# ilya16/MultINN

Hardware: AMD Instinct MI355X
Metric: piano-roll timesteps/sec (train step), 5-track LSTM-NADE (higher is better)
Workload: dtype fp16; 1 GPU; TGT joint LSTM-NADE [1024,256,88,5]; global_batch=1024, per_gpu_batch=1024, seq_len=256, pitches=88, tracks=5, nade_hidden=256, optimizer=TF-Adam lr 0.01 eps 1e-4 clip 5.0, parallelism=dp1

## Files before the change

multinn_amd/csrc/nade_mfma.hip:

```cpp
#include "common.h"
#include "lstm_handoff.h"
typedef float nm_f4 __attribute__((ext_vector_type(4)));
#define NM_ST4(dst, a) __builtin_nontemporal_store((nm_f4){a[0], a[1], a[2], a[3]}, reinterpret_cast<nm_f4*>(dst))
#define NM_ST1(dst, x) __builtin_nontemporal_store((float)(x), dst)
#include <algorithm>
#include <type_traits>

typedef __bf16 bf16x8_t __attribute__((ext_vector_type(8)));
typedef float f32x4_t __attribute__((ext_vector_type(4)));
typedef __attribute__((address_space(1))) const void* gas_ptr_t;
typedef __attribute__((address_space(3))) void* lds_ptr_t;

#ifdef NM_TRACE
__device__ long long nm_trace[16];
#define NM_T(k) do { if (tid == 0 && blockIdx.x == NM_TRACE) { const long long now_ = wall_clock64(); nm_trace[k] += now_ - tprev_; tprev_ = now_; } } while (0)
#else
#define NM_T(k) do { } while (0)
#endif
#define NADE_EPS 1e-6f
#define LN2F 0.6931471805599453f
#define NM_H 256
#define NM_PITCH 264
#define NM_LP 36

__device__ __forceinline__ float nm_ln(float x) { return __builtin_amdgcn_logf(x) * LN2F; }

typedef _Float16 f16x8_t __attribute__((ext_vector_type(8)));
struct NmPairB { f16x8_t hi, lo; };
template <bool SPLIT> struct NmState;
template <> struct NmState<false> { typedef bf16_t T; static constexpr int PITCH = NM_PITCH; };
template <> struct NmState<true> { typedef unsigned T; static constexpr int PITCH = 260; };
__device__ __forceinline__ unsigned nm_pack_hl(float x) {
    const float hi = __uint_as_float(__float_as_uint(x) & 0xFFFFE000u);
    return __builtin_bit_cast(unsigned, __builtin_amdgcn_cvt_pkrtz(hi, x - hi));
}

template <bool SPLIT>
struct NadeFwdSmemT {
    float sA[SPLIT ? 1 : 32][NM_H];
    typename NmState<SPLIT>::T sH[32][NmState<SPLIT>::PITCH];
    typename NmState<SPLIT>::T sF[32][NmState<SPLIT>::PITCH];
    float sLb[32][NM_LP];
    float sLf[32][NM_LP];
    unsigned sMask[2][32];
    unsigned sSb[2][33];
    unsigned short sFl[2][1024];
    unsigned short sPs[2][34];
    unsigned sAct[2][32];
};

__device__ __forceinline__ void nm_load_a(const bf16_t (*tile)[NM_PITCH], int mi, int lane, bf16x8_t (&a)[8]) {
    const bf16_t* p = &tile[16 * mi + (lane & 15)][8 * (lane >> 4)];
#pragma unroll
    for (int s = 0; s < 8; ++s) a[s] = *reinterpret_cast<const bf16x8_t*>(p + 32 * s);
}
template <bool SPLIT> __device__ __forceinline__ typename NmState<SPLIT>::T nm_state(float h) {
    if constexpr (SPLIT) return nm_pack_hl(h);
    else return f32_to_bf16(h);
}
__device__ __forceinline__ f32x4_t nm_dot(const bf16x8_t (&af)[8], const bf16x8_t (&bfr)[8]) {
    f32x4_t acc = {0.f, 0.f, 0.f, 0.f};
#pragma unroll
    for (int s = 0; s < 8; ++s) acc = __builtin_amdgcn_mfma_f32_16x16x32_bf16(af[s], bfr[s], acc, 0, 0, 0);
    return acc;
}
__device__ __forceinline__ f32x4_t nm_dot_hl(const unsigned (*tile)[260], int mi, int lane, const NmPairB (&bw)[8]) {
    const unsigned* p = &tile[16 * mi + (lane & 15)][8 * (lane >> 4)];
    f32x4_t accm = {0.f, 0.f, 0.f, 0.f}, accs = {0.f, 0.f, 0.f, 0.f};
#pragma unroll
    for (int s = 0; s < 8; ++s) {
        const uint4 q0 = *reinterpret_cast<const uint4*>(p + 32 * s), q1 = *reinterpret_cast<const uint4*>(p + 32 * s + 4);
        uint4 uh, ul;
        uh.x = __builtin_amdgcn_perm(q0.y, q0.x, 0x05040100u); ul.x = __builtin_amdgcn_perm(q0.y, q0.x, 0x07060302u);
        uh.y = __builtin_amdgcn_perm(q0.w, q0.z, 0x05040100u); ul.y = __builtin_amdgcn_perm(q0.w, q0.z, 0x07060302u);
        uh.z = __builtin_amdgcn_perm(q1.y, q1.x, 0x05040100u); ul.z = __builtin_amdgcn_perm(q1.y, q1.x, 0x07060302u);
        uh.w = __builtin_amdgcn_perm(q1.w, q1.z, 0x05040100u); ul.w = __builtin_amdgcn_perm(q1.w, q1.z, 0x07060302u);
        const f16x8_t ah = __builtin_bit_cast(f16x8_t, uh), al = __builtin_bit_cast(f16x8_t, ul);
        accs = __builtin_amdgcn_mfma_f32_16x16x32_f16(ah, bw[s].lo, accs, 0, 0, 0);
        accm = __builtin_amdgcn_mfma_f32_16x16x32_f16(ah, bw[s].hi, accm, 0, 0, 0);
        accs = __builtin_amdgcn_mfma_f32_16x16x32_f16(al, bw[s].hi, accs, 0, 0, 0);
    }
    return accm + accs;
}
template <bool SPLIT, typename Tile, typename B>
__device__ __forceinline__ void nm_logit_tile(const Tile& tile, int w, int lane, const B& bfr, float (*out)[NM_LP]) {
    const int ni = w >> 1, mi = w & 1;
    f32x4_t acc;
    if constexpr (SPLIT) {
        acc = nm_dot_hl(tile, mi, lane, bfr);
    } else {
        bf16x8_t af[8];
        nm_load_a(tile, mi, lane, af);
        acc = nm_dot(af, bfr);
    }
#pragma unroll
    for (int i = 0; i < 4; ++i) out[16 * mi + 4 * (lane >> 4) + i][16 * ni + (lane & 15)] = acc[i];
}

template <bool SPLIT>
__device__ __forceinline__ void
nade_fwd_mfma_body(int tracks, int N, int D, const uint8_t* __restrict__ v, long v_track_stride, const float* __restrict__ bias, int ld_bias,
                     const float* __restrict__ w_enc, const bf16_t* __restrict__ w_dec_bf, const float* __restrict__ row_weight,
                     float* __restrict__ nll, float* __restrict__ cond_p, float* __restrict__ d_bias, float* __restrict__ a_final,
                     const int* __restrict__ gate, int run_if, const int* __restrict__ n_rows_dev) {
    extern __shared__ __attribute__((aligned(16))) char smem_raw[];
    typedef NadeFwdSmemT<SPLIT> NadeFwdSmem;
    typedef typename NmState<SPLIT>::T state_t;
    typedef typename std::conditional<SPLIT, NmPairB, bf16x8_t>::type bfrag_t;
    constexpr int KS = 8;
    NadeFwdSmem& S = *reinterpret_cast<NadeFwdSmem*>(smem_raw);
    if (gate != nullptr && *gate != run_if) return;
    constexpr int Hn = NM_H;
    const int m = blockIdx.y;
    const int tid = threadIdx.x, lane = tid & 63, w = __builtin_amdgcn_readfirstlane(tid >> 6);
    const int ni = w >> 1;
    const int rb = blockIdx.x * 32;
    const uint8_t* __restrict__ vm = v + (size_t)m * v_track_stride;
    const float* __restrict__ we = w_enc + (size_t)m * D * Hn;
    const bf16_t* __restrict__ wd = w_dec_bf + (size_t)m * D * Hn * (SPLIT ? 2 : 1);
    const int bd_off = tracks * Hn + m * D;
    const int ntile = (D + 31) / 32;
    if (n_rows_dev != nullptr && rb >= *n_rows_dev) {
        if (d_bias != nullptr)
            for (int e = tid; e < 32 * D; e += 256) {
                const int n = e / D, i = e - n * D;
                if (rb + n < N) d_bias[(size_t)(rb + n) * ld_bias + bd_off + i] = 0.f;
            }
        if (nll != nullptr && tid < 32 && rb + tid < N) nll[(size_t)m * N + rb + tid] = 0.f;
        return;
    }

    float areg[SPLIT ? 32 : 1];
    {
        float av[32];
#pragma unroll
        for (int n = 0; n < 32; ++n) av[n] = bias[(size_t)min(rb + n, N - 1) * ld_bias + m * Hn + tid];
#pragma unroll
        for (int n = 0; n < 32; ++n) {
            const float x = rb + n < N ? av[n] : 0.f;
            if constexpr (SPLIT) areg[n] = x;
            else S.sA[n][tid] = x;
            S.sH[n][tid] = nm_state<SPLIT>(fast_sigmoid(x));
        }
    }
    auto load_v = [&](int c, unsigned char (&vb)[4]) {
#pragma unroll
        for (int i = 0; i < 4; ++i) {
            const int row = min(rb + 8 * w + 2 * i + (lane >> 5), N - 1), dd = min(32 * c + (lane & 31), D - 1);
            vb[i] = vm[(size_t)row * D + dd];
        }
    };
    auto ballots = [&](int c, const unsigned char (&vb)[4], unsigned (&msk)[32]) {
#pragma unroll
        for (int i = 0; i < 4; ++i) {
            const int row = rb + 8 * w + 2 * i + (lane >> 5), dd = 32 * c + (lane & 31);
            const unsigned long long bal = __ballot(row < N && dd < D && vb[i] != 0);
            if (lane == 0) { msk[8 * w + 2 * i] = (unsigned)bal; msk[8 * w + 2 * i + 1] = (unsigned)(bal >> 32); }
        }
    };
    auto build_list = [&](int buf) {
        if (w == 0) {
            const unsigned mk = lane < 32 ? S.sMask[buf][lane] : 0u;
            const int cnt = __popc(mk);
            unsigned rest = mk;
            int base = 0;
            for (int j = 0; j < 32; ++j) {
                const unsigned act = (unsigned)__ballot(cnt > j);
                if (lane == 0) { S.sPs[buf][j] = (unsigned short)base; S.sAct[buf][j] = act; }
                if (act == 0u) break;
                if (cnt > j) {
                    const int pos = base + __popc(act & ((1u << lane) - 1u));
                    const int dpos = __builtin_ctz(rest);
                    rest &= rest - 1;
                    S.sFl[buf][pos] = (unsigned short)((lane << 5) | dpos);
                }
                base += __popc(act);
            }
            if (lane == 0) S.sSb[buf][32] = (unsigned)base;
        }
    };
    auto load_b = [&](int c, bfrag_t (&b)[KS]) {
        const int d = min(32 * c + 16 * ni + (lane & 15), D - 1);
        if constexpr (SPLIT) {
            const f16_t* p = reinterpret_cast<const f16_t*>(wd) + (size_t)d * 2 * Hn + 8 * (lane >> 4);
#pragma unroll
            for (int s = 0; s < KS; ++s) {
                b[s].hi = *reinterpret_cast<const f16x8_t*>(p + 32 * s);
                b[s].lo = *reinterpret_cast<const f16x8_t*>(p + Hn + 32 * s);
            }
        } else {
            const bf16_t* p = wd + (size_t)d * Hn + 8 * (lane >> 4);
#pragma unroll
            for (int s = 0; s < KS; ++s) b[s] = *reinterpret_cast<const bf16x8_t*>(p + 32 * s);
        }
    };
    const __amdgpu_buffer_rsrc_t we_rs = __builtin_amdgcn_make_buffer_rsrc(const_cast<float*>(we), 0, D * Hn * 4, 0x00020000);
    auto load_we = [&](int c, int buf, int k0, float (&wv)[32]) {
        const int F = (int)S.sSb[buf][32];
        const int entv = (int)S.sFl[buf][(k0 + (lane & 31) < F) ? k0 + (lane & 31) : 0];
#pragma unroll
        for (int u = 0; u < 32; ++u) {
            const int e = __builtin_amdgcn_readlane(entv, u);
            wv[u] = __builtin_bit_cast(float, __builtin_amdgcn_raw_buffer_load_b32(we_rs, tid * 4, min(32 * c + (e & 31), D - 1) * (Hn * 4), 0));
        }
    };
    unsigned char vb[4];
    bfrag_t bfr[KS];
    float wev[32];
    load_v(0, vb);
    load_b(0, bfr);
    ballots(0, vb, S.sMask[0]);
    if (ntile > 1) load_v(1, vb);
    __syncthreads();
    build_list(0);
    __syncthreads();
    load_we(0, 0, 0, wev);

    const int en = tid >> 3, ed0 = 4 * (tid & 7), erow = rb + en;
    const bool evalid = erow < N;
    const int err = evalid ? erow : N - 1;
    const float rw = (row_weight != nullptr && evalid) ? row_weight[erow] : 0.f;
    float lp = 0.f;
#ifdef NM_TRACE
    long long tprev_ = wall_clock64();
#endif
    for (int c = 0; c < ntile; ++c) {
        const int buf = c & 1, nbuf = buf ^ 1;
        float bdec[4];
        {
            const float* bp = bias + (size_t)err * ld_bias + bd_off + 32 * c + ed0;
            if (32 * c + ed0 + 3 < D && (((size_t)bp) & 15) == 0) {
                const float4 b4 = *reinterpret_cast<const float4*>(bp);
                bdec[0] = b4.x; bdec[1] = b4.y; bdec[2] = b4.z; bdec[3] = b4.w;
            } else {
#pragma unroll
                for (int k = 0; k < 4; ++k) bdec[k] = bias[(size_t)err * ld_bias + bd_off + min(32 * c + ed0 + k, D - 1)];
            }
        }
        __builtin_amdgcn_sched_barrier(0);
        nm_logit_tile<SPLIT>(S.sH, w, lane, bfr, S.sLb);
        if (c + 1 < ntile) {
            ballots(c + 1, vb, S.sMask[nbuf]);
            if (c + 2 < ntile) load_v(c + 2, vb);
        }
        NM_T(0);
        hf_lds_barrier();
        NM_T(1);
        const int F = (int)S.sSb[buf][32];
        const unsigned mk = S.sMask[buf][en];
        float lsel[4];
        int jj[4];
#pragma unroll
        for (int k = 0; k < 4; ++k) {
            jj[k] = __popc(mk & ((1u << (ed0 + k)) - 1u));
            lsel[k] = S.sLb[en][ed0 + k];
        }
        int slot_of[4];
#pragma unroll
        for (int k = 0; k < 4; ++k) {
            const int pj = max(jj[k] - 1, 0);
            slot_of[k] = jj[k] > 0 ? (int)S.sPs[buf][pj] + __popc(S.sAct[buf][pj] & ((1u << en) - 1u)) : -1;
        }
        for (int k0 = 0; k0 < F; k0 += 32) {
            if (k0 > 0) load_we(c, buf, k0, wev);
            const int cnt = min(32, F - k0);
            const int flv = (int)S.sFl[buf][min(k0 + (lane & 31), F - 1)];
#pragma unroll
            for (int u0 = 0; u0 < 32; u0 += 8) {
                if (u0 < cnt) {
                    int n[8];
#pragma unroll
                    for (int i = 0; i < 8; ++i) n[i] = __builtin_amdgcn_readlane(flv, u0 + i) >> 5;
                    if constexpr (SPLIT) {
                        float x[8];
#pragma unroll
                        for (int i = 0; i < 8; ++i) {
                            x[i] = areg[n[i]] + ((u0 + i < cnt) ? wev[u0 + i] : 0.f);
                            areg[n[i]] = x[i];
                        }
                        state_t hb[8];
#pragma unroll
                        for (int i = 0; i < 8; ++i) hb[i] = nm_state<SPLIT>(fast_sigmoid(x[i]));
#pragma unroll
                        for (int i = 0; i < 8; ++i) {
                            if (u0 + i < cnt) {
                                S.sF[u0 + i][tid] = hb[i];
                                S.sH[n[i]][tid] = hb[i];
                            }
                        }
                    } else {
                        bool indep = u0 + 8 <= cnt;
#pragma unroll
                        for (int i = 0; i < 7; ++i) indep = indep && n[i] < n[i + 1];
                        if (indep) {
                            float x[8];
#pragma unroll
                            for (int i = 0; i < 8; ++i) x[i] = S.sA[n[i]][tid];
#pragma unroll
                            for (int i = 0; i < 8; ++i) x[i] += wev[u0 + i];
                            state_t hb[8];
#pragma unroll
                            for (int i = 0; i < 8; ++i) hb[i] = nm_state<SPLIT>(fast_sigmoid(x[i]));
#pragma unroll
                            for (int i = 0; i < 8; ++i) {
                                S.sA[n[i]][tid] = x[i];
                                S.sF[u0 + i][tid] = hb[i];
                                S.sH[n[i]][tid] = hb[i];
                            }
                        } else {
#pragma unroll
                            for (int i = 0; i < 8; ++i) {
                                if (u0 + i < cnt) {
                                    const float av = S.sA[n[i]][tid] + wev[u0 + i];
                                    S.sA[n[i]][tid] = av;
                                    const state_t hb1 = nm_state<SPLIT>(fast_sigmoid(av));
                                    S.sF[u0 + i][tid] = hb1;
                                    S.sH[n[i]][tid] = hb1;
                                }
                            }
                        }
                    }
                }
            }
            NM_T(2);
            if (k0 == 0 && c + 1 < ntile) build_list(nbuf);
            NM_T(3);
            hf_lds_barrier();
            NM_T(4);
            nm_logit_tile<SPLIT>(S.sF, w, lane, bfr, S.sLf);
            if (k0 == 0 && F <= 32 && c + 1 < ntile) load_we(c + 1, nbuf, 0, wev);
            NM_T(5);
            hf_lds_barrier();
            NM_T(6);
#pragma unroll
            for (int k = 0; k < 4; ++k) {
                const int slot = slot_of[k] - k0;
                if (slot_of[k] >= 0 && slot >= 0 && slot < 32) lsel[k] = S.sLf[slot][ed0 + k];
            }
        }
        if (F == 0 && c + 1 < ntile) {
            build_list(nbuf);
            hf_lds_barrier();
            load_we(c + 1, nbuf, 0, wev);
        } else if (F > 32 && c + 1 < ntile) {
            load_we(c + 1, nbuf, 0, wev);
        }
#pragma unroll
        for (int k = 0; k < 4; ++k) asm volatile("" :: "v"(bdec[k]));
        if (c + 1 < ntile) load_b(c + 1, bfr);
        NM_T(7);
        float prv[4], dbv[4];
#pragma unroll
        for (int k = 0; k < 4; ++k) {
            const int dpos = ed0 + k, gd = 32 * c + dpos;
            prv[k] = 0.f; dbv[k] = 0.f;
            if (gd >= D) continue;
            const float l = bdec[k] + lsel[k];
            const bool on = (mk >> dpos) & 1u;
            const float pr = fast_sigmoid(l);
            const float qr = fast_sigmoid(-l);
            lp += on ? nm_ln(NADE_EPS + pr) : nm_ln(NADE_EPS + qr);
            prv[k] = pr;
            const float dnll_dp = on ? -fast_rcp(NADE_EPS + pr) : fast_rcp(NADE_EPS + qr);
            dbv[k] = rw * dnll_dp * pr * qr;
        }
        if (evalid) {
            const int gd0 = 32 * c + ed0;
            const bool full = gd0 + 3 < D;
            if (cond_p != nullptr) {
                float* dst = cond_p + ((size_t)m * N + erow) * D + gd0;
                if (full && (((size_t)dst) & 15) == 0) NM_ST4(dst, prv);
                else {
#pragma unroll
                    for (int k = 0; k < 4; ++k) if (gd0 + k < D) dst[k] = prv[k];
                }
            }
            if (d_bias != nullptr) {
                float* dst = d_bias + (size_t)erow * ld_bias + bd_off + gd0;
                if (full && (((size_t)dst) & 15) == 0) NM_ST4(dst, dbv);
                else {
#pragma unroll
                    for (int k = 0; k < 4; ++k) if (gd0 + k < D) dst[k] = dbv[k];
                }
            }
        }
        NM_T(8);
    }
    lp += __shfl_xor(lp, 1);
    lp += __shfl_xor(lp, 2);
    lp += __shfl_xor(lp, 4);
    if ((tid & 7) == 0 && evalid && nll != nullptr) nll[(size_t)m * N + erow] = -lp;
    if (a_final != nullptr) {
#pragma unroll
        for (int n = 0; n < 32; ++n)
            if (rb + n < N) NM_ST1(&a_final[((size_t)m * N + rb + n) * Hn + tid], SPLIT ? areg[SPLIT ? n : 0] : S.sA[SPLIT ? 0 : n][tid]);
    }
}

template <bool SPLIT> __global__ void nade_fwd_mfma_kernel(int, int, int, const uint8_t*, long, const float*, int, const float*, const bf16_t*, const float*,
                                                           float*, float*, float*, float*, const int*, int, const int*);
template <>
__global__ void __launch_bounds__(256)
nade_fwd_mfma_kernel<false>(int tracks, int N, int D, const uint8_t* __restrict__ v, long v_track_stride, const float* __restrict__ bias, int ld_bias,
                            const float* __restrict__ w_enc, const bf16_t* __restrict__ w_dec_bf, const float* __restrict__ row_weight,
                            float* __restrict__ nll, float* __restrict__ cond_p, float* __restrict__ d_bias, float* __restrict__ a_final,
                            const int* __restrict__ gate, int run_if, const int* __restrict__ n_rows_dev) {
    nade_fwd_mfma_body<false>(tracks, N, D, v, v_track_stride, bias, ld_bias, w_enc, w_dec_bf, row_weight, nll, cond_p, d_bias, a_final, gate, run_if, n_rows_dev);
}
template <>
__global__ void __launch_bounds__(256) __attribute__((amdgpu_waves_per_eu(2, 2)))
nade_fwd_mfma_kernel<true>(int tracks, int N, int D, const uint8_t* __restrict__ v, long v_track_stride, const float* __restrict__ bias, int ld_bias,
                           const float* __restrict__ w_enc, const bf16_t* __restrict__ w_dec_bf, const float* __restrict__ row_weight,
                           float* __restrict__ nll, float* __restrict__ cond_p, float* __restrict__ d_bias, float* __restrict__ a_final,
                           const int* __restrict__ gate, int run_if, const int* __restrict__ n_rows_dev) {
    nade_fwd_mfma_body<true>(tracks, N, D, v, v_track_stride, bias, ld_bias, w_enc, w_dec_bf, row_weight, nll, cond_p, d_bias, a_final, gate, run_if, n_rows_dev);
}

extern "C" int mnn_nade_mfma_ok(int Hn) { return Hn == NM_H ? 1 : 0; }

extern "C" int mnn_nade_logprob_fwd_mfma(mnn_stream_t s, int tracks, int N, int D, int Hn, const uint8_t* v, long v_track_stride,
                                         const float* bias, int ld_bias, const float* w_enc, const void* w_dec_bf16, const float* row_weight,
                                         float* nll, float* cond_p, float* d_bias, float* a_final) {
    return mnn_nade_logprob_fwd_mfma_gated(s, tracks, N, D, Hn, v, v_track_stride, bias, ld_bias, w_enc, w_dec_bf16, row_weight, nll, cond_p, d_bias,
                                           a_final, nullptr, 0, nullptr);
}

template <bool SPLIT>
static int nm_launch(mnn_stream_t s, int tracks, int N, int D, int Hn, const uint8_t* v, long v_track_stride, const float* bias, int ld_bias,
                     const float* w_enc, const void* w_dec16, const float* row_weight, float* nll, float* cond_p, float* d_bias, float* a_final,
                     const int* gate, int run_if, const int* n_rows_dev) {
    MNN_REQUIRE(tracks > 0 && N > 0 && D > 0 && Hn == NM_H, "mnn_nade_logprob_fwd_mfma: need tracks,N,D>0 and Hn == 256 (Hn=%d)", Hn);
    MNN_REQUIRE(v && bias && w_enc && w_dec16, "mnn_nade_logprob_fwd_mfma: null pointer");
    MNN_REQUIRE(ld_bias >= tracks * (Hn + D), "mnn_nade_logprob_fwd_mfma: ld_bias %d < tracks*(Hn+D)", ld_bias);
    MNN_REQUIRE(d_bias == nullptr || row_weight != nullptr, "mnn_nade_logprob_fwd_mfma: d_bias needs row_weight");
    MNN_REQUIRE(((uintptr_t)w_dec16 & 15) == 0, "mnn_nade_logprob_fwd_mfma: the 16-bit decoder weights must be 16-byte aligned");
    static MnnPerDeviceOnce raised;
    MNN_HIP(mnn_once_per_device(raised, [] { return mnn_raise_dynamic_lds((const void*)nade_fwd_mfma_kernel<SPLIT>, (int)sizeof(NadeFwdSmemT<SPLIT>)); }));
    dim3 grid(cdiv(N, 32), tracks);
    hipLaunchKernelGGL(nade_fwd_mfma_kernel<SPLIT>, grid, dim3(256), sizeof(NadeFwdSmemT<SPLIT>), (hipStream_t)s, tracks, N, D, v, v_track_stride, bias,
                       ld_bias, w_enc, (const bf16_t*)w_dec16, row_weight, nll, cond_p, d_bias, a_final, gate, run_if, n_rows_dev);
    MNN_LAUNCH_CHECK();
    return MNN_OK;
}

extern "C" int mnn_nade_logprob_fwd_mfma_gated(mnn_stream_t s, int tracks, int N, int D, int Hn, const uint8_t* v, long v_track_stride,
                                               const float* bias, int ld_bias, const float* w_enc, const void* w_dec_bf16, const float* row_weight,
                                               float* nll, float* cond_p, float* d_bias, float* a_final, const int* gate, int run_if, const int* n_rows_dev) {
    return nm_launch<false>(s, tracks, N, D, Hn, v, v_track_stride, bias, ld_bias, w_enc, w_dec_bf16, row_weight, nll, cond_p, d_bias, a_final, gate, run_if, n_rows_dev);
}

extern "C" int mnn_nade_logprob_fwd_mfma_f32(mnn_stream_t s, int tracks, int N, int D, int Hn, const uint8_t* v, long v_track_stride,
                                             const float* bias, int ld_bias, const float* w_enc, const void* w_dec_packed, const float* row_weight,
                                             float* nll, float* cond_p, float* d_bias, float* a_final, const int* gate, int run_if, const int* n_rows_dev) {
    return nm_launch<true>(s, tracks, N, D, Hn, v, v_track_stride, bias, ld_bias, w_enc, w_dec_packed, row_weight, nll, cond_p, d_bias, a_final, gate, run_if, n_rows_dev);
}

__global__ void __launch_bounds__(256) nade_f32_pack_kernel(const float* __restrict__ w, long n, int Hn, float* __restrict__ out) {
    f16_t* o = reinterpret_cast<f16_t*>(out);
    for (long e = blockIdx.x * 256L + threadIdx.x; e < n; e += (long)gridDim.x * 256) {
        const long row = e / Hn;
        const int k = (int)(e - row * Hn);
        const float x = w[e];
        const f16_t hi = (f16_t)x;
        o[row * 2 * Hn + k] = hi;
        o[row * 2 * Hn + Hn + k] = (f16_t)(x - (float)hi);
    }
}
extern "C" int mnn_nade_f32_pack(mnn_stream_t s, const float* w_dec, long rows, int Hn, float* out) {
    MNN_REQUIRE(w_dec && out && rows > 0 && Hn > 0 && Hn % 8 == 0, "mnn_nade_f32_pack: bad arguments (Hn must be a multiple of 8)");
    MNN_REQUIRE(((uintptr_t)out & 15) == 0, "mnn_nade_f32_pack: the packed buffer must be 16-byte aligned");
    const long n = rows * Hn;
    hipLaunchKernelGGL(nade_f32_pack_kernel, dim3((int)std::min(2048L, (n + 255) / 256)), dim3(256), 0, (hipStream_t)s, w_dec, n, Hn, out);
    MNN_LAUNCH_CHECK();
    return MNN_OK;
}
```

Measured before the change: 20.58 million timesteps/s.

## Give each wave its own rows and active-pitch list, keep pre-activations in registers

```diff
diff --git a/multinn_amd/csrc/nade_mfma.hip b/multinn_amd/csrc/nade_mfma.hip
--- a/multinn_amd/csrc/nade_mfma.hip
+++ b/multinn_amd/csrc/nade_mfma.hip
@@ -2,7 +2,6 @@
 #include "lstm_handoff.h"
 typedef float nm_f4 __attribute__((ext_vector_type(4)));
 #define NM_ST4(dst, a) __builtin_nontemporal_store((nm_f4){a[0], a[1], a[2], a[3]}, reinterpret_cast<nm_f4*>(dst))
-#define NM_ST1(dst, x) __builtin_nontemporal_store((float)(x), dst)
 #include <algorithm>
 #include <type_traits>
 
@@ -37,16 +36,14 @@
 
 template <bool SPLIT>
 struct NadeFwdSmemT {
-    float sA[SPLIT ? 1 : 32][NM_H];
     typename NmState<SPLIT>::T sH[32][NmState<SPLIT>::PITCH];
     typename NmState<SPLIT>::T sF[32][NmState<SPLIT>::PITCH];
     float sLb[32][NM_LP];
     float sLf[32][NM_LP];
     unsigned sMask[2][32];
-    unsigned sSb[2][33];
-    unsigned short sFl[2][1024];
-    unsigned short sPs[2][34];
-    unsigned sAct[2][32];
+    unsigned sSb[2][32];
+    unsigned sCnt[2][4];
+    unsigned char sFl[2][4][256];
 };
 
 __device__ __forceinline__ void nm_load_a(const bf16_t (*tile)[NM_PITCH], int mi, int lane, bf16x8_t (&a)[8]) {
@@ -97,6 +94,9 @@
     for (int i = 0; i < 4; ++i) out[16 * mi + 4 * (lane >> 4) + i][16 * ni + (lane & 15)] = acc[i];
 }
 
+#define NM_P 12
+typedef float nm_f2 __attribute__((ext_vector_type(2)));
+typedef float nm_f4u __attribute__((ext_vector_type(4), aligned(4)));
 template <bool SPLIT>
 __device__ __forceinline__ void
 nade_fwd_mfma_body(int tracks, int N, int D, const uint8_t* __restrict__ v, long v_track_stride, const float* __restrict__ bias, int ld_bias,
@@ -105,9 +105,11 @@
                      const int* __restrict__ gate, int run_if, const int* __restrict__ n_rows_dev) {
     extern __shared__ __attribute__((aligned(16))) char smem_raw[];
     typedef NadeFwdSmemT<SPLIT> NadeFwdSmem;
-    typedef typename NmState<SPLIT>::T state_t;
+    typedef typename std::conditional<SPLIT, uint4, ushort4>::type state4_t;
     typedef typename std::conditional<SPLIT, NmPairB, bf16x8_t>::type bfrag_t;
     constexpr int KS = 8;
+    constexpr int P = NM_P;
+    static_assert(P % 4 == 0 && P <= 16, "the prefetched rows are handled four at a time; their list entries sit in lanes 0..15");
     NadeFwdSmem& S = *reinterpret_cast<NadeFwdSmem*>(smem_raw);
     if (gate != nullptr && *gate != run_if) return;
     constexpr int Hn = NM_H;
@@ -130,17 +132,26 @@
         return;
     }
 
-    float areg[SPLIT ? 32 : 1];
+    auto state4 = [&](const float (&x)[4]) {
+        state4_t h;
+        h.x = nm_state<SPLIT>(fast_sigmoid(x[0])); h.y = nm_state<SPLIT>(fast_sigmoid(x[1]));
+        h.z = nm_state<SPLIT>(fast_sigmoid(x[2])); h.w = nm_state<SPLIT>(fast_sigmoid(x[3]));
+        return h;
+    };
+    unsigned long long a01[8], a23[8];
+    auto pair_of = [](float lo, float hi) { return __builtin_bit_cast(unsigned long long, (nm_f2){lo, hi}); };
     {
-        float av[32];
-#pragma unroll
-        for (int n = 0; n < 32; ++n) av[n] = bias[(size_t)min(rb + n, N - 1) * ld_bias + m * Hn + tid];
-#pragma unroll
-        for (int n = 0; n < 32; ++n) {
-            const float x = rb + n < N ? av[n] : 0.f;
-            if constexpr (SPLIT) areg[n] = x;
-            else S.sA[n][tid] = x;
-            S.sH[n][tid] = nm_state<SPLIT>(fast_sigmoid(x));
+        nm_f4 av[8];
+#pragma unroll
+        for (int r = 0; r < 8; ++r)
+            av[r] = *reinterpret_cast<const nm_f4u*>(&bias[(size_t)min(rb + 8 * w + r, N - 1) * ld_bias + m * Hn + 4 * lane]);
+#pragma unroll
+        for (int r = 0; r < 8; ++r) {
+            float x[4];
+#pragma unroll
+            for (int q = 0; q < 4; ++q) x[q] = rb + 8 * w + r < N ? av[r][q] : 0.f;
+            a01[r] = pair_of(x[0], x[1]); a23[r] = pair_of(x[2], x[3]);
+            *reinterpret_cast<state4_t*>(&S.sH[8 * w + r][4 * lane]) = state4(x);
         }
     }
     auto load_v = [&](int c, unsigned char (&vb)[4]) {
@@ -150,34 +161,23 @@
             vb[i] = vm[(size_t)row * D + dd];
         }
     };
-    auto ballots = [&](int c, const unsigned char (&vb)[4], unsigned (&msk)[32]) {
+    auto ballots = [&](int c, const unsigned char (&vb)[4], int b) {
+        int cum = 0;
 #pragma unroll
         for (int i = 0; i < 4; ++i) {
             const int row = rb + 8 * w + 2 * i + (lane >> 5), dd = 32 * c + (lane & 31);
-            const unsigned long long bal = __ballot(row < N && dd < D && vb[i] != 0);
-            if (lane == 0) { msk[8 * w + 2 * i] = (unsigned)bal; msk[8 * w + 2 * i + 1] = (unsigned)(bal >> 32); }
-        }
-    };
-    auto build_list = [&](int buf) {
-        if (w == 0) {
-            const unsigned mk = lane < 32 ? S.sMask[buf][lane] : 0u;
-            const int cnt = __popc(mk);
-            unsigned rest = mk;
-            int base = 0;
-            for (int j = 0; j < 32; ++j) {
-                const unsigned act = (unsigned)__ballot(cnt > j);
-                if (lane == 0) { S.sPs[buf][j] = (unsigned short)base; S.sAct[buf][j] = act; }
-                if (act == 0u) break;
-                if (cnt > j) {
-                    const int pos = base + __popc(act & ((1u << lane) - 1u));
-                    const int dpos = __builtin_ctz(rest);
-                    rest &= rest - 1;
-                    S.sFl[buf][pos] = (unsigned short)((lane << 5) | dpos);
-                }
-                base += __popc(act);
-            }
-            if (lane == 0) S.sSb[buf][32] = (unsigned)base;
-        }
+            const bool on = row < N && dd < D && vb[i] != 0;
+            const unsigned long long bal = __ballot(on);
+            const unsigned lo = (unsigned)bal, hi = (unsigned)(bal >> 32);
+            if ((lane & 31) == 0) {
+                S.sMask[b][8 * w + 2 * i + (lane >> 5)] = lane ? hi : lo;
+                S.sSb[b][8 * w + 2 * i + (lane >> 5)] = (unsigned)(cum + (lane ? __popc(lo) : 0));
+            }
+            if (on) S.sFl[b][w][cum + (int)__builtin_amdgcn_mbcnt_hi(hi, __builtin_amdgcn_mbcnt_lo(lo, 0u))] = (unsigned char)(64 * i + lane);
+            cum += __popcll(bal);
+        }
+        if (lane == 0) S.sCnt[b][w] = (unsigned)cum;
+        return cum;
     };
     auto load_b = [&](int c, bfrag_t (&b)[KS]) {
         const int d = min(32 * c + 16 * ni + (lane & 15), D - 1);
@@ -195,26 +195,28 @@
         }
     };
     const __amdgpu_buffer_rsrc_t we_rs = __builtin_amdgcn_make_buffer_rsrc(const_cast<float*>(we), 0, D * Hn * 4, 0x00020000);
-    auto load_we = [&](int c, int buf, int k0, float (&wv)[32]) {
-        const int F = (int)S.sSb[buf][32];
-        const int entv = (int)S.sFl[buf][(k0 + (lane & 31) < F) ? k0 + (lane & 31) : 0];
-#pragma unroll
-        for (int u = 0; u < 32; ++u) {
-            const int e = __builtin_amdgcn_readlane(entv, u);
-            wv[u] = __builtin_bit_cast(float, __builtin_amdgcn_raw_buffer_load_b32(we_rs, tid * 4, min(32 * c + (e & 31), D - 1) * (Hn * 4), 0));
+    auto load_we = [&](int c, int b, int j0, int jend, nm_f4 (&wv)[P]) {
+        const int entv = (int)S.sFl[b][w][min(j0 + (lane & 15), 255)];
+#pragma unroll
+        for (int g = 0; g < P; g += 4) {
+            if (j0 + g < jend) {
+#pragma unroll
+                for (int u = g; u < g + 4; ++u) {
+                    const int e = __builtin_amdgcn_readlane(entv, u);
+                    wv[u] = __builtin_bit_cast(nm_f4, __builtin_amdgcn_raw_buffer_load_b128(we_rs, lane * 16, min(32 * c + (e & 31), D - 1) * (Hn * 4), 0));
+                }
+            }
         }
     };
     unsigned char vb[4];
     bfrag_t bfr[KS];
-    float wev[32];
+    nm_f4 wev[P];
     load_v(0, vb);
     load_b(0, bfr);
-    ballots(0, vb, S.sMask[0]);
+    int nxt_cnt = ballots(0, vb, 0);
     if (ntile > 1) load_v(1, vb);
+    load_we(0, 0, 0, nxt_cnt, wev);
     __syncthreads();
-    build_list(0);
-    __syncthreads();
-    load_we(0, 0, 0, wev);
 
     const int en = tid >> 3, ed0 = 4 * (tid & 7), erow = rb + en;
     const bool evalid = erow < N;
@@ -240,95 +242,59 @@
         __builtin_amdgcn_sched_barrier(0);
         nm_logit_tile<SPLIT>(S.sH, w, lane, bfr, S.sLb);
         if (c + 1 < ntile) {
-            ballots(c + 1, vb, S.sMask[nbuf]);
+            nxt_cnt = ballots(c + 1, vb, nbuf);
             if (c + 2 < ntile) load_v(c + 2, vb);
         }
         NM_T(0);
         hf_lds_barrier();
         NM_T(1);
-        const int F = (int)S.sSb[buf][32];
+        const int cntv = (int)S.sCnt[buf][lane & 3];
+        const int c0 = __builtin_amdgcn_readlane(cntv, 0), c1 = __builtin_amdgcn_readlane(cntv, 1), c2 = __builtin_amdgcn_readlane(cntv, 2),
+                  c3 = __builtin_amdgcn_readlane(cntv, 3);
+        const int F = c0 + c1 + c2 + c3;
+        const int wbase = (w > 0 ? c0 : 0) + (w > 1 ? c1 : 0) + (w > 2 ? c2 : 0);
+        const int wcnt = w == 0 ? c0 : w == 1 ? c1 : w == 2 ? c2 : c3;
         const unsigned mk = S.sMask[buf][en];
+        const int sb = wbase + (int)S.sSb[buf][en];
         float lsel[4];
-        int jj[4];
+        int slot_of[4];
 #pragma unroll
         for (int k = 0; k < 4; ++k) {
-            jj[k] = __popc(mk & ((1u << (ed0 + k)) - 1u));
+            const int jj = __popc(mk & ((1u << (ed0 + k)) - 1u));
+            slot_of[k] = jj > 0 ? sb + jj - 1 : -1;
             lsel[k] = S.sLb[en][ed0 + k];
         }
-        int slot_of[4];
-#pragma unroll
-        for (int k = 0; k < 4; ++k) {
-            const int pj = max(jj[k] - 1, 0);
-            slot_of[k] = jj[k] > 0 ? (int)S.sPs[buf][pj] + __popc(S.sAct[buf][pj] & ((1u << en) - 1u)) : -1;
-        }
         for (int k0 = 0; k0 < F; k0 += 32) {
-            if (k0 > 0) load_we(c, buf, k0, wev);
-            const int cnt = min(32, F - k0);
-            const int flv = (int)S.sFl[buf][min(k0 + (lane & 31), F - 1)];
-#pragma unroll
-            for (int u0 = 0; u0 < 32; u0 += 8) {
-                if (u0 < cnt) {
-                    int n[8];
-#pragma unroll
-                    for (int i = 0; i < 8; ++i) n[i] = __builtin_amdgcn_readlane(flv, u0 + i) >> 5;
-                    if constexpr (SPLIT) {
-                        float x[8];
-#pragma unroll
-                        for (int i = 0; i < 8; ++i) {
-                            x[i] = areg[n[i]] + ((u0 + i < cnt) ? wev[u0 + i] : 0.f);
-                            areg[n[i]] = x[i];
-                        }
-                        state_t hb[8];
-#pragma unroll
-                        for (int i = 0; i < 8; ++i) hb[i] = nm_state<SPLIT>(fast_sigmoid(x[i]));
-#pragma unroll
-                        for (int i = 0; i < 8; ++i) {
+            const int jhi = min(k0 + 32 - wbase, wcnt);
+            for (int jb = max(k0 - wbase, 0); jb < jhi; jb += P) {
+                if (jb > 0) load_we(c, buf, jb, jhi, wev);
+                const int cnt = jhi - jb;
+                const int flv = (int)S.sFl[buf][w][min(jb + (lane & 15), jhi - 1)];
+#pragma unroll
+                for (int u0 = 0; u0 < P; u0 += 4) {
+                    if (u0 < cnt) {
+#pragma unroll
+                        for (int i = 0; i < 4; ++i) {
                             if (u0 + i < cnt) {
-                                S.sF[u0 + i][tid] = hb[i];
-                                S.sH[n[i]][tid] = hb[i];
-                            }
-                        }
-                    } else {
-                        bool indep = u0 + 8 <= cnt;
-#pragma unroll
-                        for (int i = 0; i < 7; ++i) indep = indep && n[i] < n[i + 1];
-                        if (indep) {
-                            float x[8];
-#pragma unroll
-                            for (int i = 0; i < 8; ++i) x[i] = S.sA[n[i]][tid];
-#pragma unroll
-                            for (int i = 0; i < 8; ++i) x[i] += wev[u0 + i];
-                            state_t hb[8];
-#pragma unroll
-                            for (int i = 0; i < 8; ++i) hb[i] = nm_state<SPLIT>(fast_sigmoid(x[i]));
-#pragma unroll
-                            for (int i = 0; i < 8; ++i) {
-                                S.sA[n[i]][tid] = x[i];
-                                S.sF[u0 + i][tid] = hb[i];
-                                S.sH[n[i]][tid] = hb[i];
-                            }
-                        } else {
-#pragma unroll
-                            for (int i = 0; i < 8; ++i) {
-                                if (u0 + i < cnt) {
-                                    const float av = S.sA[n[i]][tid] + wev[u0 + i];
-                                    S.sA[n[i]][tid] = av;
-                                    const state_t hb1 = nm_state<SPLIT>(fast_sigmoid(av));
-                                    S.sF[u0 + i][tid] = hb1;
-                                    S.sH[n[i]][tid] = hb1;
-                                }
+                                const int r = __builtin_amdgcn_readlane(flv, u0 + i) >> 5;
+                                const nm_f2 p01 = __builtin_bit_cast(nm_f2, a01[r]), p23 = __builtin_bit_cast(nm_f2, a23[r]);
+                                const float x[4] = {p01[0] + wev[u0 + i][0], p01[1] + wev[u0 + i][1], p23[0] + wev[u0 + i][2], p23[1] + wev[u0 + i][3]};
+                                a01[r] = pair_of(x[0], x[1]); a23[r] = pair_of(x[2], x[3]);
+                                __builtin_amdgcn_sched_barrier(0);
+                                const state4_t hb = state4(x);
+                                *reinterpret_cast<state4_t*>(&S.sF[wbase + jb + u0 + i - k0][4 * lane]) = hb;
+                                *reinterpret_cast<state4_t*>(&S.sH[8 * w + r][4 * lane]) = hb;
                             }
                         }
                     }
                 }
             }
             NM_T(2);
-            if (k0 == 0 && c + 1 < ntile) build_list(nbuf);
             NM_T(3);
             hf_lds_barrier();
             NM_T(4);
             nm_logit_tile<SPLIT>(S.sF, w, lane, bfr, S.sLf);
-            if (k0 == 0 && F <= 32 && c + 1 < ntile) load_we(c + 1, nbuf, 0, wev);
+            if (k0 + 32 >= F && c + 1 < ntile) load_we(c + 1, nbuf, 0, nxt_cnt, wev);
             NM_T(5);
             hf_lds_barrier();
             NM_T(6);
@@ -339,11 +305,8 @@
             }
         }
         if (F == 0 && c + 1 < ntile) {
-            build_list(nbuf);
             hf_lds_barrier();
-            load_we(c + 1, nbuf, 0, wev);
-        } else if (F > 32 && c + 1 < ntile) {
-            load_we(c + 1, nbuf, 0, wev);
+            load_we(c + 1, nbuf, 0, nxt_cnt, wev);
         }
 #pragma unroll
         for (int k = 0; k < 4; ++k) asm volatile("" :: "v"(bdec[k]));
@@ -392,8 +355,10 @@
     if ((tid & 7) == 0 && evalid && nll != nullptr) nll[(size_t)m * N + erow] = -lp;
     if (a_final != nullptr) {
 #pragma unroll
-        for (int n = 0; n < 32; ++n)
-            if (rb + n < N) NM_ST1(&a_final[((size_t)m * N + rb + n) * Hn + tid], SPLIT ? areg[SPLIT ? n : 0] : S.sA[SPLIT ? 0 : n][tid]);
+        for (int r = 0; r < 8; ++r)
+            if (rb + 8 * w + r < N)
+                __builtin_nontemporal_store(__builtin_shufflevector(__builtin_bit_cast(nm_f2, a01[r]), __builtin_bit_cast(nm_f2, a23[r]), 0, 1, 2, 3),
+                                            reinterpret_cast<nm_f4u*>(&a_final[((size_t)m * N + rb + 8 * w + r) * Hn + 4 * lane]));
     }
 }
 
@@ -434,6 +399,7 @@
     MNN_REQUIRE(ld_bias >= tracks * (Hn + D), "mnn_nade_logprob_fwd_mfma: ld_bias %d < tracks*(Hn+D)", ld_bias);
     MNN_REQUIRE(d_bias == nullptr || row_weight != nullptr, "mnn_nade_logprob_fwd_mfma: d_bias needs row_weight");
     MNN_REQUIRE(((uintptr_t)w_dec16 & 15) == 0, "mnn_nade_logprob_fwd_mfma: the 16-bit decoder weights must be 16-byte aligned");
+    static_assert(sizeof(NadeFwdSmemT<SPLIT>) <= 80 * 1024, "two workgroups share a CU's 160 KB of LDS");
     static MnnPerDeviceOnce raised;
     MNN_HIP(mnn_once_per_device(raised, [] { return mnn_raise_dynamic_lds((const void*)nade_fwd_mfma_kernel<SPLIT>, (int)sizeof(NadeFwdSmemT<SPLIT>)); }));
     dim3 grid(cdiv(N, 32), tracks);
```

Result: faster. 21.05 million timesteps/s (median of 6 runs) (+2.3%).
